# ARISE-Initiative/robosuite

Measured on AMD Instinct MI355X. Metric: env-steps/sec (whole node), Lift/Panda/OSC_POSE @4096 envs/GPU, higher is better.
Workload: dtype f32

## Files before the change

include/rsim.h:

```cpp
#ifndef RSIM_H
#define RSIM_H
#include <stddef.h>
#include <stdint.h>

#ifdef __cplusplus
extern "C" {
#endif

typedef struct rsim_model rsim_model;
typedef struct rsim_batch rsim_batch;

enum rsim_ctrl_type { RSIM_CTRL_OSC_POSE = 0, RSIM_CTRL_OSC_POSITION = 1, RSIM_CTRL_JOINT_POSITION = 2, RSIM_CTRL_JOINT_TORQUE = 3, RSIM_CTRL_JOINT_VELOCITY = 4 };
#define RSIM_JNT_MAX 16
typedef struct rsim_ctrl_desc {
  int32_t ndof;
  int32_t qpos_idx[RSIM_JNT_MAX];
  int32_t dof_idx[RSIM_JNT_MAX];
  int32_t act_idx[RSIM_JNT_MAX];
  int32_t eef_site;
  int32_t base_site;
  float kp[RSIM_JNT_MAX];
  float damping_ratio;
  float input_min[RSIM_JNT_MAX], input_max[RSIM_JNT_MAX], output_min[RSIM_JNT_MAX], output_max[RSIM_JNT_MAX];
  int32_t uncouple_pos_ori;
// ... 113 lines not shown
int rsim_sync(rsim_batch* b);
int rsim_observe(rsim_batch* b);

int rsim_set_episode(rsim_batch* b, int horizon);
int rsim_set_reset_bank(rsim_batch* b, int n_episodes, int n_patch, const int32_t* patch_idx, const float* bank);
int rsim_refill_reset_bank(rsim_batch* b, int n, const int32_t* env, const int32_t* episode, const float* rows);
int rsim_bank_poll_begin(rsim_batch* b);
int rsim_bank_poll(rsim_batch* b, int32_t* ep_index, int wait);
int rsim_refill_reset_bank_async(rsim_batch* b, int n, const int32_t* env, const int32_t* episode, const float* rows);
int rsim_bank_flush(rsim_batch* b);
int rsim_param_offset(const rsim_batch* b, const char* field, int elem);

int rsim_set_schedule(rsim_batch* b, int longest_first);
int rsim_set_applied_forces(rsim_batch* b, int enable);
int rsim_set_early_end(rsim_batch* b, int rules, int min_steps);
int rsim_end_episodes(rsim_batch* b, const uint8_t* mask_dev);
int rsim_set_stream_groups(rsim_batch* b, int groups);
void* rsim_group_stream(rsim_batch* b, int group);

int rsim_profile(rsim_batch* b, int enable, unsigned long long* out, int n_out);
int rsim_wavelog(rsim_batch* b, unsigned long long* out);
int rsim_profile_env(rsim_batch* b, int env);
int rsim_tier_snapshot(rsim_batch* b, int* host_tier);
const char* rsim_tuning_defaults(void);
int rsim_tier_stats(rsim_batch* b, unsigned long long* out2);
int rsim_pairlog(rsim_batch* b, unsigned long long* out);

int rsim_get_array(rsim_batch* b, int field, void* host_dst, size_t count);
int rsim_set_array(rsim_batch* b, int field, const void* host_src, size_t count);
void* rsim_device_ptr(rsim_batch* b, int field, size_t* count);
void* rsim_stream(rsim_batch* b);

int rsim_jac_site(rsim_batch* b, int env, int site, double* jacp, double* jacr);
int rsim_jac_body(rsim_batch* b, int env, int body, double* jacp, double* jacr);

int rsim_full_M(rsim_batch* b, int env, double* M);
typedef struct rsim_contact {
  double dist, pos[3], frame[9], friction[5], normal_force;
  int32_t geom1, geom2, dim, efc_address;
} rsim_contact;
int rsim_contacts(rsim_batch* b, int env, int max_out, rsim_contact* out);

int rsim_model_param_set(rsim_batch* b, const char* field, int env0, int nenv, const double* values, size_t count_per_env);

int rsim_model_param_get(rsim_batch* b, const char* field, int env0, int nenv, double* values, size_t count_per_env);

// ... 25 lines not shown
```

robosuite_amd/backend.py:

```python
from __future__ import annotations

import ctypes as C
import os

import numpy as np

from . import mjcf

_HERE = os.path.dirname(os.path.abspath(__file__))
LIB_PATH = os.environ.get("RSIM_LIB", os.path.join(_HERE, "librsim_hip.so"))
_LIB = None

FIELDS = ["qpos", "qvel", "qacc_warmstart", "ctrl", "time", "cstate", "xpos", "xquat", "qM", "qfrc_bias", "qfrc_passive", "qfrc_actuator",
          "qfrc_constraint", "qacc", "cdof", "rootcom", "contact", "efc_force", "ncon", "nefc", "niter", "obs", "reward", "success", "done", "ep_step",
          "ep_index", "diverged", "overflow", "bank_stale", "terminal_obs", "sensordata", "task_object", "cap_need", "qfrc_applied", "polish",
          "xfrc_applied"]
EXTRA_FIELDS = ["end_reason"]
FIELD_ID = {n: i for i, n in enumerate(FIELDS + EXTRA_FIELDS)}
END_REASONS = {"running": 0, "horizon": 1, "success": 2, "diverged": 3, "requested": 4}
INT_FIELDS = {"end_reason", "polish", "ncon", "nefc", "niter", "success", "done", "ep_step", "ep_index", "diverged", "overflow", "bank_stale", "task_object", "cap_need"}
CON_REC = 24
CSTATE = 32
OBS_MAX = 128
OBS_KINDS = {"qpos": 0, "cos": 1, "sin": 2, "qvel": 3, "qacc": 4, "site_pos": 5, "body_quat": 6, "site_quat": 7, "body_pos": 8, "body_minus_site": 9, "body_minus_body": 10,
# ... 195 lines not shown
        L.rsim_get_array.argtypes = [vp, C.c_int, vp, C.c_size_t]
        L.rsim_set_array.argtypes = [vp, C.c_int, vp, C.c_size_t]
        L.rsim_device_ptr.restype = vp
        L.rsim_device_ptr.argtypes = [vp, C.c_int, C.POINTER(C.c_size_t)]
        L.rsim_stream.restype = vp
        L.rsim_stream.argtypes = [vp]
        L.rsim_jac_site.argtypes = [vp, C.c_int, C.c_int, vp, vp]
        L.rsim_jac_body.argtypes = [vp, C.c_int, C.c_int, vp, vp]
        L.rsim_model_param_set.argtypes = [vp, C.c_char_p, C.c_int, C.c_int, vp, C.c_size_t]
        L.rsim_model_param_get.argtypes = [vp, C.c_char_p, C.c_int, C.c_int, vp, C.c_size_t]
        L.rsim_profile.argtypes = [vp, C.c_int, vp, C.c_int]
        L.rsim_wavelog.argtypes = [vp, vp]
        L.rsim_pairlog.argtypes = [vp, vp]
        L.rsim_set_schedule.argtypes = [vp, C.c_int]
        L.rsim_set_applied_forces.argtypes = [vp, C.c_int]
        L.rsim_set_stream_groups.argtypes = [vp, C.c_int]
        if hasattr(L, "rsim_set_early_end"):
            L.rsim_set_early_end.argtypes = [vp, C.c_int, C.c_int]
            L.rsim_end_episodes.argtypes = [vp, vp]
        L.rsim_group_stream.restype = vp; L.rsim_group_stream.argtypes = [vp, C.c_int]
        L.rsim_profile_env.argtypes = [vp, C.c_int]
        L.rsim_tier_snapshot.argtypes = [vp, vp]
        L.rsim_tier_stats.argtypes = [vp, vp]
        L.rsim_tuning_defaults.restype = C.c_char_p
        L.rsim_name2id.argtypes = [vp, C.c_char_p, C.c_char_p]
        L.rsim_id2name.argtypes = [vp, C.c_char_p, C.c_int]; L.rsim_id2name.restype = C.c_char_p
        L.rsim_full_M.argtypes = [vp, C.c_int, vp]
        L.rsim_contacts.argtypes = [vp, C.c_int, C.c_int, vp]
        L.rsim_comm_unique_id.argtypes = [vp, C.c_size_t]
        L.rsim_comm_create.argtypes = [vp, C.c_size_t, C.c_int, C.c_int, C.c_int, C.POINTER(vp)]
        L.rsim_allreduce_stats.argtypes = [vp, vp, C.c_int, C.c_int]
        L.rsim_comm_free.argtypes = [vp]; L.rsim_comm_free.restype = None
        _LIB = L
    return _LIB


def _chk(rc):
    if rc != 0:
        raise RsimError(lib().rsim_last_error().decode())


def tuning_sha16() -> str:
    import hashlib
    return hashlib.sha256(lib().rsim_tuning_defaults()).hexdigest()[:16]


# ... 296 lines not shown
                self._held.popleft()

    def _step_streams(self):
        import torch

        key = getattr(self, "_ngroups", 1)
        if getattr(self, "_ext_key", None) != key:
            ptrs = [self.group_stream(g) for g in range(key)] if key > 1 else [self.stream()]
            self._ext, self._ext_key = [torch.cuda.ExternalStream(p, device=f"cuda:{self.device}") for p in ptrs], key
        return self._ext

    PROFILE_SLOTS = ("load", "kin", "com", "crb", "broad", "narrow", "makec", "vel", "ctrl", "act", "solve", "euler", "store",
                     "n_sub", "n_cand", "n_con", "n_efc", "n_newton", "n_ls", "boxbox", "mpr", "plane", "n_boxbox", "n_mpr", "n_support",
                     "x0", "x1", "x2", "x3", "x4", "x5", "x6", "x7", "x8", "x9")

    def profile_env(self, env=-1):
        _chk(self._L.rsim_profile_env(self.ptr, int(env)))

    def tier_snapshot(self):
        out = np.zeros(self.B, dtype=np.int32)
        _chk(self._L.rsim_tier_snapshot(self.ptr, out.ctypes.data))
        return out

    def tier_stats(self):
        out = np.zeros(2, dtype=np.uint64)
        _chk(self._L.rsim_tier_stats(self.ptr, out.ctypes.data))
        return int(out[0]), int(out[1])

    def wavelog(self):
        out = np.zeros((self.B, 8), dtype=np.uint64)
        _chk(self._L.rsim_wavelog(self.ptr, out.ctypes.data))
        return out

    def set_applied_forces(self, enable=True):
        _chk(self._L.rsim_set_applied_forces(self.ptr, int(bool(enable))))

    def set_early_end(self, success=False, diverged=False, min_steps=1):
        _chk(self._L.rsim_set_early_end(self.ptr, (1 if success else 0) | (2 if diverged else 0), int(min_steps)))

    def end_episodes(self, mask):
        import torch

        if not isinstance(mask, torch.Tensor) or not mask.is_cuda or tuple(mask.shape) != (self.B,):
            raise RsimError(f"end_episodes: mask must be a CUDA tensor of shape ({self.B},)")
        m8 = (mask != 0).to(torch.uint8).contiguous()
        ev = torch.cuda.Event()
# ... 79 lines not shown
```

robosuite_amd/csrc/rsim_api.cpp:

```cpp
#include <hip/hip_runtime.h>
#include <dlfcn.h>
#include <rccl/rccl.h>
#include <math.h>
#include <stdarg.h>
#include <stdio.h>
#include <stdlib.h>
#include <string.h>

#include <algorithm>
#include <map>
#include <string>
#include <vector>

#include "../../include/rsim.h"
#include "rsim_internal.h"

#define RSIM_NCFG 5
#define RSIM_MAX_GROUPS 32
extern "C" int rsim_launch_step_cfg0(const DModel* m, const DBatch* b, const float* actions, int n_sub, int flags, hipStream_t stream);
extern "C" int rsim_launch_ctrl_reset_cfg0(const DModel* m, const DBatch* b, const unsigned char* mask, hipStream_t stream);
extern "C" int rsim_limits_cfg0(int* lim);
extern "C" int rsim_launch_step_cfg1(const DModel* m, const DBatch* b, const float* actions, int n_sub, int flags, hipStream_t stream);
extern "C" int rsim_launch_ctrl_reset_cfg1(const DModel* m, const DBatch* b, const unsigned char* mask, hipStream_t stream);
extern "C" int rsim_limits_cfg1(int* lim);
// ... 111 lines not shown
  int* d_patch;
  float* d_ft_base;
  float* d_ft;
  float* d_ft0;
  float* d_mesh;
  unsigned char* d_mask;
  DModel dm;
  DBatch db;
  void* fptr[RSIM_FIELD_COUNT];
  size_t fcount[RSIM_FIELD_COUNT];
  int fis_int[RSIM_FIELD_COUNT];
  int lim[10];
  int cfg;
  int cs;
  int* d_order;
  unsigned* d_cost;
  void* d_cm;
  size_t cm_bytes;
  int cm_dirty;
  DCtrl cm_ctrl;
  int tier;
  int lim_w[10];
  int* d_tier[2];
  int tier_flip;
  int share_cm;
  void* d_cm_w;
  size_t cm_bytes_w;
  int* d_wlist[2];
  int* d_wcount;
  hipStream_t wstream;
  hipEvent_t wfork, wjoin;
  int have_cost;
  int* d_order2[2];
  unsigned* d_cost2[2];
  long nstep;
  int schedule;
  int applied;
  int early_rules, early_min_steps;
  int* d_end_reason;
  int* d_seen_diverged;
  int* d_end_sel;
  int ended_outside;
  int groups, ngroups, forked;
  hipStream_t gstream[RSIM_MAX_GROUPS];
  hipEvent_t gev[RSIM_MAX_GROUPS], mev;
  hipStream_t bstream;
// ... 638 lines not shown
  dm.newton_polish_tol = getenv("RSIM_POLISH_TOL") ? (float)atof(getenv("RSIM_POLISH_TOL")) : 1.0f;
  dm.newton_polish_gate = getenv("RSIM_POLISH_GATE") ? (float)atof(getenv("RSIM_POLISH_GATE")) : 0.0f;
  dm.newton_exact = getenv("RSIM_NEWTON_EXACT") ? atoi(getenv("RSIM_NEWTON_EXACT")) : 1;
  dm.newton_ng = getenv("RSIM_NEWTON_NG") ? (float)atof(getenv("RSIM_NEWTON_NG")) : RSIM_NEWTON_NG;
  if (m->multijoint) { int r = fail("rsim_batch_create: bodies with more than one joint are not supported by the fused kernel"); delete b; return r; }
  if (m->D("jnt_stiffness")) for (int j = 0; j < m->njnt; j++) if (m->D("jnt_stiffness")[j] != 0.0) {
    int r = fail("rsim_batch_create: joint %d has a spring (stiffness %g): passive joint springs are not implemented in the fused kernel (tendon springs are)", j, m->D("jnt_stiffness")[j]);
    delete b; return r;
  }

  if (m->maxcondim > 4) { int r = fail("rsim_batch_create: condim %d contacts are not supported by the compiled kernel configuration (max 4)", m->maxcondim); delete b; return r; }
  for (int j = 0; j < m->njnt; j++) if (m->I("jnt_type")[j] == 1) { int r = fail("rsim_batch_create: ball joints are not supported by the fused kernel"); delete b; return r; }
  if (dalloc(&b->d_lt, m->lanetab.size())) return 1;
  HIPCHK(hipMemcpy(b->d_lt, m->lanetab.data(), m->lanetab.size() * sizeof(int), hipMemcpyHostToDevice));
  dm.lt = b->d_lt; dm.kin_rounds = m->kin_rounds; dm.ndynroot = m->ndynroot; dm.maxcondim = m->maxcondim;
  for (int r = 0; r < RSIM_MAXDYNROOT; r++) dm.dynroot[r] = r < m->ndynroot ? m->dynroot[r] : 0;
  dm.ft0 = b->d_ft0; dm.fenv = 0;
  dm.it = b->d_it; dm.ft = b->d_ft; dm.mesh_vert = b->d_mesh; dm.fstride = b->per_env ? (int)fs : 0;
  memcpy(dm.io, m->io, sizeof(dm.io));
  memcpy(dm.fo, m->fo, sizeof(dm.fo));
  dm.ctrl = m->ctrl;
  b->cs = m->ctrl.enabled ? m->ctrl.cs_size : RSIM_CS_SIZE;
  dm.ctrl.cs_size = b->cs;
  b->tier = TIER_NONE;
  if (b->cs <= RSIM_CS_LDS && !getenv("RSIM_NO_TIERS") && b->cfg <= 3) {
    int lw[10];
    if (b->cfg <= 2) k_limits_w[b->cfg](lw);
    else k_limits[5](lw);
    if (config_holds(m, lw)) { b->tier = b->cfg <= 2 ? TIER_FUSED : TIER_LIST; memcpy(b->lim_w, lw, sizeof(lw)); }
  }
  {
    auto jg_need = [](const int* lim) -> size_t {
      if (!(lim[9] & 4)) return 0;
      return (size_t)lim[6] * (size_t)(lim[2] + 1) + ((lim[9] & 8) ? (size_t)lim[2] * (size_t)(lim[2] + 1) : 0) + ((lim[9] & 16) ? (size_t)lim[5] * 22 : 0);
    };
    size_t jgf = jg_need(b->lim);
    if (b->tier != TIER_NONE) jgf = std::max(jgf, jg_need(b->lim_w));
    b->db.jg_stride = (long long)jgf;
    if (jgf && dalloc(&b->db.jg, (size_t)B * jgf)) return 1;
  }
  b->d_tier[0] = b->d_tier[1] = nullptr; b->tier_flip = 0;
  b->share_cm = 0; b->d_cm_w = nullptr; b->cm_bytes_w = 0; b->d_wlist[0] = b->d_wlist[1] = nullptr; b->d_wcount = nullptr; b->wstream = nullptr; b->wfork = b->wjoin = nullptr;
  if (b->tier != TIER_NONE) {
    for (int k = 0; k < 2; k++) if (dalloc(&b->d_tier[k], (size_t)B)) return 1;
    if (dalloc(&b->db.tstat, (size_t)2)) return 1;
  }
// ... 269 lines not shown
  int e = rsim_launch_step_list_cfg5(&b->dm, &dw, actions, n_sub, flags, grid, stream);
  if (e) return fail("wide-tier kernel launch failed: %s", hipGetErrorString((hipError_t)e));
  return 0;
}

static int launch(rsim_batch* b, const float* actions, int n_sub, int flags) {
  const int WCN = 2 + 2 * RSIM_MAX_GROUPS;
  HIPCHK(hipSetDevice(b->device));
  if (sync_controller(b)) return 1;
  if (b->applied) flags |= RF_APPLIED;
  const bool tiered = b->tier != TIER_NONE && (flags & RF_EPISODE) && (flags & RF_CTRL) && !(flags & RF_DEBUG);
  b->db.tier_cur = tiered ? b->d_tier[b->tier_flip] : nullptr; b->db.tier_next = tiered ? b->d_tier[b->tier_flip ^ 1] : nullptr;
  const bool no_advance = b->cfg == 0 || b->cfg == 1;
  b->db.tier_up_con = getenv("RSIM_TIER_UP_CON") ? atoi(getenv("RSIM_TIER_UP_CON")) : (no_advance ? 0 : 2);
  b->db.tier_up_efc = getenv("RSIM_TIER_UP_EFC") ? atoi(getenv("RSIM_TIER_UP_EFC")) : (no_advance ? 0 : 6);
  b->db.tier_pass = tiered ? 0 : -1; b->db.wlist = nullptr; b->db.wcount = nullptr; b->db.wlist2 = nullptr; b->db.wcount2 = nullptr;
  const bool fused = tiered && b->tier == TIER_FUSED, listed = tiered && b->tier == TIER_LIST;
  if (fused) {
    b->db.tier_con = b->lim[5]; b->db.tier_efc = b->lim[6];
    if (const char* e = getenv("RSIM_FORCE_HANDOVER")) b->db.tier_pass = 100 + atoi(e);
  }
  const bool grouped = (flags & RF_EPISODE) && (flags & RF_CTRL) && b->ngroups > 1;
  const bool early = (flags & RF_EPISODE) && b->early_rules && b->db.bank;
  if (!grouped || b->cm_dirty || memcmp(&b->cm_ctrl, &b->dm.ctrl, sizeof(DCtrl))) { if (join_groups(b)) return 1; }
  if (ensure_constants(b)) return 1;
  if ((flags & RF_OBS) && !b->dm.task.enabled) return fail("the task (observation / reward epilogue) was configured after the batch was created");
  if ((flags & RF_CTRL) && !b->dm.ctrl.enabled) return fail("no controller configured (rsim_model_set_controller)");
  b->db.order = nullptr; b->db.cost = nullptr;
  if (grouped) {
    if (fork_groups(b)) return 1;
    const bool sched = b->schedule && b->d_order;
    for (int g = 0; g < b->ngroups; g++) {
      const int e0 = (int)((long long)b->B * g / b->ngroups), e1 = (int)((long long)b->B * (g + 1) / b->ngroups);
      DBatch db = b->db;
      db.env0 = e0; db.nenv = e1 - e0;
      if (sched) {
        if (b->have_cost) {
          int eo = rsim_launch_order(b->d_cost + e0, b->d_order + e0, e1 - e0, b->gstream[g]);
          if (eo) return fail("dispatch-order kernel launch failed: %s", hipGetErrorString((hipError_t)eo));
          db.order = b->d_order + e0;
        }
        db.cost = b->d_cost;
      }
      if (listed) {
        int* cnt = b->d_wcount + b->tier_flip * WCN + 2 + 2 * g;
        int el = rsim_launch_tier_list(b->db.tier_cur, b->d_wlist[0] + e0, cnt, b->d_wcount + (b->tier_flip ^ 1) * WCN + 2 + 2 * g, e0, e1 - e0, b->gstream[g]);
        if (el) return fail("tier-list kernel launch failed: %s", hipGetErrorString((hipError_t)el));
        db.wlist2 = b->d_wlist[1] + e0; db.wcount2 = cnt + 1;
      }
      int e = k_step_launch[b->cfg](&b->dm, &db, actions, n_sub, flags, b->gstream[g]);
      if (e) return fail("kernel launch failed: %s", hipGetErrorString((hipError_t)e));
      if (listed) {
        int* cnt = b->d_wcount + b->tier_flip * WCN + 2 + 2 * g;
        if (wide_pass(b, actions, n_sub, flags, 1, b->d_wlist[0] + e0, cnt, b->gstream[g])) return 1;
        if (wide_pass(b, actions, n_sub, flags, 2, b->d_wlist[1] + e0, cnt + 1, b->gstream[g])) return 1;
      }
      if (early && end_episodes_launch(b, e0, e1 - e0, nullptr, 0, (flags & (RF_APPLIED | RF_DEBUG)) ? 1 : 0, b->gstream[g])) return 1;
      if (b->db.bank && (b->db.horizon > 0 || early)) {
        db.order = nullptr; db.cost = nullptr;
        if (b->db.bank_P > 0 && b->db.cm_stride) {
          e = k_prepare_launch[b->cfg](&b->dm, &db, e1 - e0, 1, b->gstream[g]);
          if (e) return fail("constant-block kernel launch failed: %s", hipGetErrorString((hipError_t)e));
        }
        if (b->dm.task.enabled) {
          db.tier_cur = nullptr; db.tier_next = nullptr; db.tier_pass = -1; db.wlist = nullptr; db.wcount = nullptr; db.wlist2 = nullptr; db.wcount2 = nullptr;
          e = k_reset_obs_launch[b->cfg](&b->dm, &db, b->gstream[g]);
          if (e) return fail("reset-observation kernel launch failed: %s", hipGetErrorString((hipError_t)e));
        }
      }
    }
    if (sched) b->have_cost = 1;
    if (tiered) b->tier_flip ^= 1;
    b->gen++;
    b->derived_stale = 1;
    return 0;
  }
  const bool sched1 = (flags & RF_EPISODE) && (flags & RF_CTRL) && b->schedule && b->d_order;
  const int cur = (int)(b->nstep & 1), prev = cur ^ 1;
  const bool traced = sched1_trace(flags);
  if (traced) tr_mark(b, 0);
  if (sched1) {
// ... 9 lines not shown
    int* cnt = b->d_wcount + b->tier_flip * WCN;
    HIPCHK(hipEventRecord(b->wfork, b->stream));
    HIPCHK(hipStreamWaitEvent(b->wstream, b->wfork, 0));
    int el = rsim_launch_tier_list(b->db.tier_cur, b->d_wlist[0], cnt, b->d_wcount + (b->tier_flip ^ 1) * WCN, 0, b->B, b->wstream);
    if (el) return fail("tier-list kernel launch failed: %s", hipGetErrorString((hipError_t)el));
    if (wide_pass(b, actions, n_sub, flags, 1, b->d_wlist[0], cnt, b->wstream)) return 1;
    HIPCHK(hipEventRecord(b->wjoin, b->wstream));
    b->db.wlist2 = b->d_wlist[1]; b->db.wcount2 = cnt + 1;
  }
  if (traced) tr_mark(b, 2);
  int e = k_step_launch[b->cfg](&b->dm, &b->db, actions, n_sub, flags, b->stream);
  if (e) return fail("kernel launch failed: %s", hipGetErrorString((hipError_t)e));
  if (traced) tr_mark(b, 3);
  if (listed) {
    HIPCHK(hipStreamWaitEvent(b->stream, b->wjoin, 0));
    if (traced) tr_mark(b, 4);
    if (wide_pass(b, actions, n_sub, flags, 2, b->d_wlist[1], b->d_wcount + b->tier_flip * WCN + 1, b->stream)) return 1;
  } else if (traced) tr_mark(b, 4);
  if (tiered) b->tier_flip ^= 1;
  if (traced) tr_mark(b, 5);
  if (sched1) b->nstep++;
  if (early && end_episodes_launch(b, 0, b->B, nullptr, 0, (flags & (RF_APPLIED | RF_DEBUG)) ? 1 : 0, b->stream)) return 1;
  if ((flags & RF_EPISODE) && b->db.bank && (b->db.horizon > 0 || early)) {
    if (b->db.bank_P > 0 && b->db.cm_stride) {
      e = k_prepare_launch[b->cfg](&b->dm, &b->db, b->B, 1, b->stream);
      if (e) return fail("constant-block kernel launch failed: %s", hipGetErrorString((hipError_t)e));
    }
    if (traced) tr_mark(b, 6);
    if (b->dm.task.enabled) {
      DBatch db2 = b->db;
      db2.order = nullptr; db2.cost = nullptr;
      db2.tier_cur = nullptr; db2.tier_next = nullptr; db2.tier_pass = -1; db2.wlist = nullptr; db2.wcount = nullptr; db2.wlist2 = nullptr; db2.wcount2 = nullptr;
      e = k_reset_obs_launch[b->cfg](&b->dm, &db2, b->stream);
      if (e) return fail("reset-observation kernel launch failed: %s", hipGetErrorString((hipError_t)e));
    }
    if (traced) tr_mark(b, 7);
  }
  b->gen++;
  b->derived_stale = (flags & RF_DEBUG) ? 0 : 1;
  return 0;
}
static bool derived_field(int f) { return (f >= RSIM_XPOS && f <= RSIM_NITER) || f == RSIM_SENSORDATA; }
extern "C" int rsim_forward(rsim_batch* b);
static int refresh_forward(rsim_batch* b) {
  DBatch keep = b->db;
  b->db.overflow = nullptr; b->db.cap_need = nullptr; b->db.mprc = nullptr; b->db.bpl = nullptr;
  const int r = launch(b, nullptr, 1, RF_POSVEL | RF_ACTSOLVE | RF_DEBUG | RF_NOSTORE);
  b->db.overflow = keep.overflow; b->db.cap_need = keep.cap_need; b->db.mprc = keep.mprc; b->db.bpl = keep.bpl;
  return r;
}
static int refresh_derived(rsim_batch* b, int field) { return (derived_field(field) && b->derived_stale) ? refresh_forward(b) : 0; }
extern "C" int rsim_forward(rsim_batch* b) { return launch(b, nullptr, 1, RF_POSVEL | RF_ACTSOLVE | RF_DEBUG); }
// ... 300 lines not shown
  static const char* const envs[] = {"RSIM_NEWTON_NS", "RSIM_NEWTON_NA", "RSIM_NEWTON_LS", "RSIM_NEWTON_NG", "RSIM_NEWTON_WIDE", "RSIM_NEWTON_EXACT", "RSIM_NEWTON_REFINE",
                                     "RSIM_POLISH_TOL", "RSIM_POLISH_GATE", "RSIM_BP_REACH", "RSIM_NEAR_THRESH", "RSIM_NEAR_GAIN", "RSIM_MPR_CONE", "RSIM_NO_MPR_WARMSTART", "RSIM_NO_MPR_PORTAL_WARMSTART",
                                     "RSIM_TIER_UP_CON", "RSIM_TIER_UP_EFC", "RSIM_NO_TIERS", "RSIM_NO_SHARE_CM", "RSIM_EULER_FULL", "RSIM_FORCE_HANDOVER"};
  for (const char* e : envs) if (const char* v = getenv(e)) { s += ";env:"; s += e; s += "="; s += v; }
  return s.c_str();
}
extern "C" int rsim_tier_stats(rsim_batch* b, unsigned long long* out2) {
  if (!out2) return fail("rsim_tier_stats: null destination");
  out2[0] = out2[1] = 0;
  if (b->tier == TIER_NONE) return 0;
  HIPCHK(hipSetDevice(b->device));
  if (join_groups(b)) return 1;
  HIPCHK(hipStreamSynchronize(b->stream));
  HIPCHK(hipMemcpy(out2, b->db.tstat, 2 * sizeof(unsigned long long), hipMemcpyDeviceToHost));
  return 0;
}
extern "C" int rsim_tier_snapshot(rsim_batch* b, int* host_tier) {
  if (!host_tier) return fail("rsim_tier_snapshot: null destination");
  HIPCHK(hipSetDevice(b->device));
  if (b->tier == TIER_NONE) { memset(host_tier, 0, (size_t)b->B * sizeof(int)); return 0; }
  if (join_groups(b)) return 1;
  HIPCHK(hipStreamSynchronize(b->stream));
  HIPCHK(hipMemcpy(host_tier, b->d_tier[b->tier_flip], (size_t)b->B * sizeof(int), hipMemcpyDeviceToHost));
  return 0;
}

extern "C" int rsim_wavelog(rsim_batch* b, unsigned long long* out) { if (join_groups(b)) return 1;
  if (!b->db.prof) return fail("rsim_wavelog: profiling is not enabled");
  HIPCHK(hipSetDevice(b->device));
  HIPCHK(hipStreamSynchronize(b->stream));
  HIPCHK(hipMemcpy(out, b->db.prof + RP_COUNT, 8 * (size_t)b->B * sizeof(unsigned long long), hipMemcpyDeviceToHost));
  return 0;
}

extern "C" void* rsim_device_ptr(rsim_batch* b, int field, size_t* count) {
  if (field < 0 || field >= RSIM_FIELD_COUNT) { fail("bad field id %d", field); return nullptr; }
  if (count) *count = b->fcount[field];
  if (refresh_derived(b, field)) return nullptr;
  return b->fptr[field];
}
extern "C" int rsim_get_array(rsim_batch* b, int field, void* dst, size_t count) { if (join_groups(b)) return 1;
  if (field < 0 || field >= RSIM_FIELD_COUNT) return fail("bad field id %d", field);
  if (count > b->fcount[field]) return fail("rsim_get_array: count %zu > field size %zu", count, b->fcount[field]);
  if (refresh_derived(b, field)) return 1;
  HIPCHK(hipSetDevice(b->device));
  HIPCHK(hipStreamSynchronize(b->stream));
// ... 272 lines not shown
```

robosuite_amd/csrc/rsim_internal.h:

```cpp
#pragma once
#include <stdint.h>

enum {
  IO_body_parentid, IO_body_rootid, IO_body_jntadr, IO_body_jntnum, IO_body_dofadr, IO_body_dofnum, IO_body_depth,
  IO_body_mocap, IO_body_moving, IO_body_ancmask , IO_body_dofmask , IO_body_isroot,
  IO_jnt_type, IO_jnt_qposadr, IO_jnt_dofadr, IO_jnt_bodyid, IO_jnt_limited,
  IO_dof_bodyid, IO_dof_jntid, IO_dof_ancmask , IO_dof_cvelmask , IO_dof_zerodot,
  IO_cg_geomid, IO_cg_type, IO_cg_bodyid, IO_cg_condim, IO_cg_priority, IO_cg_meshadr, IO_cg_meshnum,
  IO_pair_g1, IO_pair_g2,
  IO_site_bodyid,
  IO_act_trnid, IO_act_biastype, IO_act_ctrllimited, IO_act_forcelimited,
  IO_tendon_adr, IO_tendon_num, IO_tendon_limited, IO_wrap_dof, IO_wrap_qadr, IO_eq_tendon,
  IO_sensor_type , IO_sensor_site, IO_sensor_adr ,
  IO_COUNT
};
enum {
  FO_body_pos, FO_body_quat, FO_body_ipos, FO_body_iquat, FO_body_mass, FO_body_inertia, FO_body_invweight0, FO_body_subtreemass,
  FO_jnt_pos, FO_jnt_axis, FO_jnt_range, FO_jnt_margin, FO_jnt_solref, FO_jnt_solimp, FO_qpos0,
  FO_dof_armature, FO_dof_damping, FO_dof_frictionloss, FO_dof_solref, FO_dof_solimp, FO_dof_invweight0,
  FO_cg_size, FO_cg_pos, FO_cg_quat, FO_cg_friction, FO_cg_solref, FO_cg_solimp, FO_cg_solmix, FO_cg_margin, FO_cg_gap,
  FO_cg_rbound, FO_cg_rcenter, FO_cg_aabb ,
  FO_cg_capsule ,
  FO_site_pos, FO_site_quat,
  FO_act_gear, FO_act_gainprm, FO_act_biasprm, FO_act_ctrlrange, FO_act_forcerange,
// ... 191 lines not shown
#define RSIM_NEWTON_NA 1e-5f
#define RSIM_NEWTON_NG 0.f
#endif

enum { RP_LOAD, RP_KIN, RP_COM, RP_CRB, RP_BROAD, RP_NARROW, RP_MAKEC, RP_VEL, RP_CTRL, RP_ACT, RP_SOLVE, RP_EULER, RP_STORE,
       RP_N_SUB, RP_N_CAND, RP_N_CON, RP_N_EFC, RP_N_NEWTON, RP_N_LS, RP_BOXBOX, RP_MPR, RP_PLANE, RP_N_BOXBOX, RP_N_MPR, RP_N_SUPPORT,
       RP_X0, RP_X1, RP_X2, RP_X3, RP_X4, RP_X5, RP_X6, RP_X7, RP_X8, RP_X9,  RP_COUNT };

struct DDr { float density, viscosity, pos, quat, inertia, mass, friction, solref, solimp, frictionloss, damping, armature;
             unsigned long long body_mask, geom_mask, joint_mask; };

enum {
  RF_POSVEL = 1,
  RF_CTRL = 2,
  RF_SETGOAL = 4,
  RF_ACTSOLVE = 8,
  RF_INTEGRATE = 16,
  RF_DEBUG = 32,
  RF_OBS = 64,
  RF_EPISODE = 128,
  RF_RESET_ONLY = 256,
  RF_NOSTORE = 512,
  RF_APPLIED = 1024,
};
```

robosuite_amd/csrc/rsim_step.hip:

```cpp
#include <hip/hip_runtime.h>
#include <stdint.h>
#include <type_traits>

#include "../../include/rsim.h"
#include "rsim_internal.h"

#ifndef RSIM_CFG
#define RSIM_CFG 0
#endif
#if RSIM_CFG == 0
#define RSIM_DIMS 32, 16, 16, 24, 16, 16, 64, 192
#define RSIM_SYM(x) x##_cfg0
#define RSIM_DIMS_W 32, 16, 16, 24, 16, 32, 128, 192
#elif RSIM_CFG == 1
#define RSIM_DIMS 32, 16, 32, 24, 16, 32, 64, 192
#define RSIM_SYM(x) x##_cfg1
#define RSIM_DIMS_W 32, 16, 32, 24, 16, 32, 128, 192
#elif RSIM_CFG == 2
#define RSIM_DIMS 64, 16, 16, 32, 32, 32, 64, 320
#define RSIM_SYM(x) x##_cfg2
#define RSIM_DIMS_W 64, 16, 16, 32, 32, 32, 128, 320
#elif RSIM_CFG == 3
#define RSIM_DIMS 64, 32, 48, 64, 32, 32, 128, 640
#define RSIM_SYM(x) x##_cfg3
// ... 3874 lines not shown
      }
      if (lane == 0 && t.task == 1) {
        const V3 cube = ld3(sm.xpos + 3 * t.object_body), grip = ld3(sm.spos + 3 * t.grip_site);
        const bool succ = cube.z > t.table_height + t.lift_margin;
        float r = 0.f;
        if (succ) r = 2.25f;
        else if (t.reward_shaping) { r = 1.f - tanhf(10.f * norm(cube - grip)); if (grasp) r += 0.25f; }
        if (reward) { *reward = r * t.reward_scale / 2.25f; *success = succ ? 1 : 0; }
      }
    }
  }

  __device__ __forceinline__ void fwd_constraint() {
    if (sm.nefc == 0) {
      if (lane < m.nv) { sm.qacc[lane] = sm.qacc_smooth[lane]; sm.qfrc_constraint[lane] = 0.f; }
      if (lane == 0) sm.niter = 0;
      SYNC();
      return;
    }
    solve_newton();
  }
};

struct Handover { int sub0; float time; bool fresh_ctrl, handed; int ndiverged, need_con, need_efc; float cstate; unsigned t_launch; };

template <int NB, int NJ, int NV, int NG, int NS, int NCON, int NEFC, int NPAIR, bool DBG, int FUSED = 0>
__device__ __forceinline__ bool step_body(const DModel& m, const DBatch& b, const float* __restrict__ actions, int n_sub, int flags, int slot, Handover* ho = nullptr) {
  typedef Smem<NB, NJ, NV, NG, NS, NCON, NEFC, NPAIR> SM;
  const int lane = threadIdx.x;
  const int tpass = (!DBG && b.tier_cur) ? (FUSED == 2 ? 2 : FUSED == 1 ? 0 : b.tier_pass) : -1;
  const bool resume = FUSED == 2 && ho->sub0 > 0;
  if ((tpass <= 0 || FUSED) && slot >= (b.nenv ? b.nenv : b.B)) return false;
  const int env = uni((tpass > 0 && !FUSED) ? b.wlist[slot] : (b.order ? b.order[slot] : slot) + b.env0);
  if ((flags & RF_RESET_ONLY) && !b.needs_reset[env]) return false;
  if (!FUSED && tpass == 0 && b.tier_cur[env] != 0) return false;
  const unsigned t_launch = resume ? ho->t_launch : (b.cost ? (unsigned)uni((int)(clock64() >> 6)) : 0u);
  const float* fp = m.ft + (size_t)env * m.fstride;
  Sim<SM> sim(m, fp, lane, b.prof, b.cm, b.cm_stride ? (const char*)b.cm_env + (size_t)env * b.cm_stride : (const char*)b.cm);
  sim.pf.acc = b.prof_env == -1 || b.prof_env == env;
  if (b.prof) sim.pf.pairs = b.prof + RP_COUNT + 8 * (size_t)b.B;
  sim.pf.start();
  if (b.prof && lane == 0 && !resume) {
    unsigned long long* wl = b.prof + RP_COUNT + 8 * (size_t)env;
    wl[0] = (unsigned)__builtin_amdgcn_s_getreg((31 << 11) | 4);
    wl[1] = (unsigned)__builtin_amdgcn_s_getreg((31 << 11) | 20);
    wl[2] = wall_clock64();
  }
  if (!resume) {
    for (int i = lane; i < m.nq; i += 64) sm.qpos[i] = b.qpos[(size_t)env * m.nq + i];
    for (int i = lane; i < m.nv; i += 64) { sm.qvel[i] = b.qvel[(size_t)env * m.nv + i]; sm.qacc_ws[i] = b.qacc_ws[(size_t)env * m.nv + i]; }
    if (lane >= m.nv && lane < NV) { sm.qvel[lane] = 0.f; sm.qacc_ws[lane] = 0.f; sm.qacc[lane] = 0.f; }
    for (int i = lane; i < m.nu; i += 64) sm.ctrl[i] = b.ctrl[(size_t)env * m.nu + i];
  }
  const int cs = m.ctrl.cs_size, csl = cs < RSIM_CS_LDS ? cs : RSIM_CS_LDS;
  sim.cst = (gwf)(b.cstate + (size_t)env * cs);
  if (b.bpl) sim.bpl = (int __attribute__((address_space(1)))*)(b.bpl + (size_t)env * 320);
  if (b.mprc) { sim.mprc = (gwf)(b.mprc + (size_t)env * Sim<SM>::MPRC * m.npair); sim.mpr_portal = b.mprc_portal != 0; }
  if constexpr (Sim<SM>::JG) sim.Jg = (gwf)(b.jg + (size_t)env * b.jg_stride);
  if constexpr (Sim<SM>::MG) sim.Mg = sim.Jg + SM::NEFC_ * SM::JS_;
// ... 131 lines not shown
    const bool done = b.horizon > 0 && st >= b.horizon;
    if (done && b.bank) {
      const int ep = b.ep_index[env] + 1, slot = ep % b.bank_E;
      const float* src = b.bank + ((size_t)env * b.bank_E + slot) * (m.nq + b.bank_P);
      if (lane == 0 && b.bank_tag && b.bank_tag[(size_t)env * b.bank_E + slot] != ep) b.bank_stale[env] += 1;
      if (b.term_obs && m.task.enabled) for (int i = lane; i < m.task.nobs; i += 64) b.term_obs[(size_t)env * m.task.nobs + i] = b.obs[(size_t)env * m.task.nobs + i];
      SYNC();
      for (int i = lane; i < m.nq; i += 64) sm.qpos[i] = src[i];
      if (lane < NV) { sm.qvel[lane] = 0.f; sm.qacc_ws[lane] = 0.f; sm.ctrl[lane] = 0.f; }
      for (int p2 = lane; p2 < b.bank_P; p2 += 64) {
        const int pi = b.patch_idx[p2];
        if (pi < 0) { b.task_object[env] = (int)src[m.nq + p2]; continue; }
        b.ft_rw[(size_t)env * m.fstride + pi] = src[m.nq + p2];
        if (b.ft_base) b.ft_base[(size_t)env * m.fstride + pi] = src[m.nq + p2];
      }
      time = 0.f;
      st = 0;
      if (sim.mprc) for (int p2 = lane; p2 < m.npair; p2 += 64) sim.mprc[Sim<SM>::MPRC * p2 + 3] = 0.f;
      if (DBG || (flags & RF_APPLIED)) {
        for (int i = lane; i < m.nv; i += 64) b.qfrc_applied[(size_t)env * m.nv + i] = 0.f;
        for (int i = lane; i < m.nbody * 6; i += 64) b.xfrc_applied[(size_t)env * m.nbody * 6 + i] = 0.f;
      }
      if (lane == 0) { b.ep_index[env] = ep; b.needs_reset[env] = 1; }
      SYNC();
    }
    if (lane == 0) { b.done[env] = done ? 1 : 0; b.ep_step[env] = st; }
  }
  if (!DBG || !(flags & RF_NOSTORE)) {
    for (int i = lane; i < m.nq; i += 64) b.qpos[(size_t)env * m.nq + i] = sm.qpos[i];
    for (int i = lane; i < m.nv; i += 64) { b.qvel[(size_t)env * m.nv + i] = sm.qvel[i]; b.qacc_ws[(size_t)env * m.nv + i] = sm.qacc_ws[i]; }
    for (int i = lane; i < m.nu; i += 64) b.ctrl[(size_t)env * m.nu + i] = sm.ctrl[i];
    if (lane < csl) sim.cst[lane] = sm.cstate[lane];
    if (lane == 0) b.time[env] = time;
  }
  if (b.overflow && lane == 0 && sim.ovf) b.overflow[env] += sim.ovf;
  if (b.cap_need && lane == 0) { int* cn = b.cap_need + 2 * (size_t)env; if (sim.need_con > cn[0]) cn[0] = sim.need_con; if (sim.need_efc > cn[1]) cn[1] = sim.need_efc; }
  if (b.cost && lane == 0) {
    unsigned cst = (unsigned)(clock64() >> 6) - t_launch;
    if (sim.near_sep < m.near_thresh) cst += (unsigned)((float)cst * m.near_gain);
    b.cost[env] = cst;
  }
  if (b.prof && lane == 0) {
    unsigned long long* wl = b.prof + RP_COUNT + 8 * (size_t)env;
    wl[3] = wall_clock64(); wl[4] = sim.pf.c_mpr; wl[5] = sim.pf.c_support; wl[6] = sim.pf.c_newton; wl[7] = sim.pf.c_cand;
  }
  if constexpr (DBG) if (flags & RF_DEBUG) {
    const int nb = m.nbody, nv = m.nv;
    for (int i = lane; i < nb * 3; i += 64) { b.xpos[(size_t)env * nb * 3 + i] = sm.xpos[i]; b.rootcom[(size_t)env * nb * 3 + i] = sm.rootcom[3 * sim.cm->broot[i / 3] + i % 3]; }
    for (int i = lane; i < nb * 4; i += 64) b.xquat[(size_t)env * nb * 4 + i] = sm.xquat[i];
    for (int e = lane; e < nv * nv; e += 64) { int i = e / nv, j = e - i * nv; b.qM[(size_t)env * nv * nv + e] = sim.Mrd(i * SM::NVP + j); }
    for (int e = lane; e < nv * 6; e += 64) b.cdof[(size_t)env * nv * 6 + e] = sm.cdof[(e / 6) * 9 + e % 6];
    for (int i = lane; i < nv; i += 64) {
      size_t o = (size_t)env * nv + i;
      b.qfrc_bias[o] = sm.qfrc_bias[i]; b.qfrc_passive[o] = sm.qfrc_passive[i];
      if (flags & RF_ACTSOLVE) { b.qfrc_actuator[o] = sm.qfrc_actuator[i]; b.qfrc_constraint[o] = sm.qfrc_constraint[i]; b.qacc[o] = sm.qacc[i]; }
    }
    int ncon = sm.ncon;
    sim.csync();
    for (int c = lane; c < ncon; c += 64) {
      float* r = b.contact + ((size_t)env * NCON + c) * RSIM_CON_REC;
// ... 8 lines not shown
      for (int i = lane; i < sm.nefc; i += 64) b.efc_force[(size_t)env * NEFC + i] = sm.e_force[i];
    if (lane == 0) { b.ncon[env] = ncon; b.nefc[env] = sm.nefc; b.niter[env] = sm.niter; if (b.polish) b.polish[env] = sm.polish; }
  }
  return false;
}

#ifdef RSIM_WAVES_PER_EU
#define RSIM_KSTEP_ATTR __attribute__((amdgpu_waves_per_eu(RSIM_WAVES_PER_EU, RSIM_WAVES_PER_EU)))
#else
#define RSIM_KSTEP_ATTR
#endif
template <int NB, int NJ, int NV, int NG, int NS, int NCON, int NEFC, int NPAIR>
__global__ RSIM_KSTEP_ATTR __launch_bounds__(64, RSIM_MINWAVES) void k_step(DModel m, DBatch b, const float* __restrict__ actions, int n_sub, int flags) {
#ifdef RSIM_DIMS_W
  typedef const char __attribute__((address_space(4)))* ka_t;
  ka_t ka = (ka_t)__builtin_amdgcn_kernarg_segment_ptr();
  constexpr size_t b_off = (sizeof(DModel) + alignof(DBatch) - 1) & ~(alignof(DBatch) - 1);
  const DModel& mk = *(const DModel*)(const DModel __attribute__((address_space(4)))*)ka;
  const DBatch& bk = *(const DBatch*)(const DBatch __attribute__((address_space(4)))*)(ka + b_off);
#define m mk
#define b bk
  const int slot = (int)blockIdx.x;
  Handover ho;
  ho.sub0 = 0; ho.time = 0.f; ho.fresh_ctrl = false; ho.handed = false; ho.ndiverged = 0; ho.need_con = 0; ho.need_efc = 0; ho.cstate = 0.f; ho.t_launch = 0u;
  bool wide = false;
  if (b.tier_cur) {
    if (slot >= (b.nenv ? b.nenv : b.B)) return;
    wide = b.tier_cur[uni((b.order ? b.order[slot] : slot) + b.env0)] != 0;
  }
  if (!wide) {
    const int over = uni(step_body<NB, NJ, NV, NG, NS, NCON, NEFC, NPAIR, false, 1>(m, b, actions, n_sub, flags, slot, &ho) ? 1 : 0);
    if (!over) return;
    ho.sub0 = uni(ho.sub0); ho.time = __builtin_bit_cast(float, uni(__builtin_bit_cast(int, ho.time))); ho.fresh_ctrl = uni(ho.fresh_ctrl ? 1 : 0) != 0; ho.handed = true;
    ho.ndiverged = uni(ho.ndiverged); ho.need_con = uni(ho.need_con); ho.need_efc = uni(ho.need_efc); ho.t_launch = (unsigned)uni((int)ho.t_launch);
  }
  step_body<RSIM_DIMS_W, false, 2>(m, b, actions, n_sub, flags, slot, &ho);
#undef m
#undef b
#else
  step_body<NB, NJ, NV, NG, NS, NCON, NEFC, NPAIR, false>(m, b, actions, n_sub, flags, (int)blockIdx.x);
#endif
}
template <int NB, int NJ, int NV, int NG, int NS, int NCON, int NEFC, int NPAIR>
__global__ __launch_bounds__(64, 1) void k_step_list(DModel m, DBatch b, const float* __restrict__ actions, int n_sub, int flags) {
  const int n = *b.wcount;
  for (int i = blockIdx.x; i < n; i += gridDim.x) {
    step_body<NB, NJ, NV, NG, NS, NCON, NEFC, NPAIR, false>(m, b, actions, n_sub, flags, i);
    __syncthreads();
  }
}
template <int NB, int NJ, int NV, int NG, int NS, int NCON, int NEFC, int NPAIR>
__global__ __launch_bounds__(64, 1) void k_step_dbg(DModel m, DBatch b, const float* __restrict__ actions, int n_sub, int flags) {
  step_body<NB, NJ, NV, NG, NS, NCON, NEFC, NPAIR, true>(m, b, actions, n_sub, flags, (int)blockIdx.x);
}
template <int NB, int NJ, int NV, int NG, int NS, int NCON, int NEFC, int NPAIR>
__global__ __launch_bounds__(64, 1) void k_reset_obs(DModel m, DBatch b) {
  step_body<NB, NJ, NV, NG, NS, NCON, NEFC, NPAIR, false>(m, b, nullptr, 1, RF_POSVEL | RF_ACTSOLVE | RF_OBS | RF_RESET_ONLY, (int)blockIdx.x);
}

// ... 203 lines not shown
```

Before: 1.289 million.

## Run episode reset and re-observation inside the fused step kernel

When an environment's episode restarts during the fused step, the kernel now loops back in the same workgroup. It rebuilds per-env constant blocks and re-runs a reset-only forward/observe pass, instead of the host launching separate prepare and reset kernels over the whole batch. This removes extra full-batch kernel launches and the passes that scan all environments only to act on the few being reset. It adds fences and scalar cache invalidation inside the kernel, plus extra code that may raise register pressure. An env var can restore the separate pass, and a debug API exposes the restart flags.

```diff
diff --git a/include/rsim.h b/include/rsim.h
--- a/include/rsim.h
+++ b/include/rsim.h
@@ -159,6 +159,7 @@
 int rsim_wavelog(rsim_batch* b, unsigned long long* out);
 int rsim_profile_env(rsim_batch* b, int env);
 int rsim_tier_snapshot(rsim_batch* b, int* host_tier);
+int rsim_restart_flags(rsim_batch* b, int* host_flags);
 const char* rsim_tuning_defaults(void);
 int rsim_tier_stats(rsim_batch* b, unsigned long long* out2);
 int rsim_pairlog(rsim_batch* b, unsigned long long* out);
diff --git a/robosuite_amd/backend.py b/robosuite_amd/backend.py
--- a/robosuite_amd/backend.py
+++ b/robosuite_amd/backend.py
@@ -241,6 +241,8 @@
         L.rsim_profile_env.argtypes = [vp, C.c_int]
         L.rsim_tier_snapshot.argtypes = [vp, vp]
         L.rsim_tier_stats.argtypes = [vp, vp]
+        if hasattr(L, "rsim_restart_flags"):
+            L.rsim_restart_flags.argtypes = [vp, vp]
         L.rsim_tuning_defaults.restype = C.c_char_p
         L.rsim_name2id.argtypes = [vp, C.c_char_p, C.c_char_p]
         L.rsim_id2name.argtypes = [vp, C.c_char_p, C.c_int]; L.rsim_id2name.restype = C.c_char_p
@@ -583,6 +585,11 @@
         _chk(self._L.rsim_tier_snapshot(self.ptr, out.ctypes.data))
         return out
 
+    def restart_flags(self):
+        out = np.zeros(self.B, dtype=np.int32)
+        _chk(self._L.rsim_restart_flags(self.ptr, out.ctypes.data))
+        return out
+
     def tier_stats(self):
         out = np.zeros(2, dtype=np.uint64)
         _chk(self._L.rsim_tier_stats(self.ptr, out.ctypes.data))
diff --git a/robosuite_amd/csrc/rsim_api.cpp b/robosuite_amd/csrc/rsim_api.cpp
--- a/robosuite_amd/csrc/rsim_api.cpp
+++ b/robosuite_amd/csrc/rsim_api.cpp
@@ -157,6 +157,7 @@
   int tier;
   int lim_w[10];
   int* d_tier[2];
+  int separate_reset;
   int tier_flip;
   int share_cm;
   void* d_cm_w;
@@ -841,6 +842,7 @@
   dm.ctrl = m->ctrl;
   b->cs = m->ctrl.enabled ? m->ctrl.cs_size : RSIM_CS_SIZE;
   dm.ctrl.cs_size = b->cs;
+  { const char* e = getenv("RSIM_SEPARATE_RESET_PASS"); b->separate_reset = (e && atoi(e) != 0) ? 1 : 0; }
   b->tier = TIER_NONE;
   if (b->cs <= RSIM_CS_LDS && !getenv("RSIM_NO_TIERS") && b->cfg <= 3) {
     int lw[10];
@@ -1156,6 +1158,8 @@
   }
   const bool grouped = (flags & RF_EPISODE) && (flags & RF_CTRL) && b->ngroups > 1;
   const bool early = (flags & RF_EPISODE) && b->early_rules && b->db.bank;
+  const bool inkernel = (b->lim[9] & 32) && !b->separate_reset && !early && (flags & RF_EPISODE) && (flags & RF_CTRL) && !(flags & RF_DEBUG);
+  if (inkernel) flags |= RF_RESET_INKERNEL;
   if (!grouped || b->cm_dirty || memcmp(&b->cm_ctrl, &b->dm.ctrl, sizeof(DCtrl))) { if (join_groups(b)) return 1; }
   if (ensure_constants(b)) return 1;
   if ((flags & RF_OBS) && !b->dm.task.enabled) return fail("the task (observation / reward epilogue) was configured after the batch was created");
@@ -1190,7 +1194,7 @@
         if (wide_pass(b, actions, n_sub, flags, 2, b->d_wlist[1] + e0, cnt + 1, b->gstream[g])) return 1;
       }
       if (early && end_episodes_launch(b, e0, e1 - e0, nullptr, 0, (flags & (RF_APPLIED | RF_DEBUG)) ? 1 : 0, b->gstream[g])) return 1;
-      if (b->db.bank && (b->db.horizon > 0 || early)) {
+      if (!inkernel && b->db.bank && (b->db.horizon > 0 || early)) {
         db.order = nullptr; db.cost = nullptr;
         if (b->db.bank_P > 0 && b->db.cm_stride) {
           e = k_prepare_launch[b->cfg](&b->dm, &db, e1 - e0, 1, b->gstream[g]);
@@ -1246,12 +1250,12 @@
   if (sched1) b->nstep++;
   if (early && end_episodes_launch(b, 0, b->B, nullptr, 0, (flags & (RF_APPLIED | RF_DEBUG)) ? 1 : 0, b->stream)) return 1;
   if ((flags & RF_EPISODE) && b->db.bank && (b->db.horizon > 0 || early)) {
-    if (b->db.bank_P > 0 && b->db.cm_stride) {
+    if (!inkernel && b->db.bank_P > 0 && b->db.cm_stride) {
       e = k_prepare_launch[b->cfg](&b->dm, &b->db, b->B, 1, b->stream);
       if (e) return fail("constant-block kernel launch failed: %s", hipGetErrorString((hipError_t)e));
     }
     if (traced) tr_mark(b, 6);
-    if (b->dm.task.enabled) {
+    if (!inkernel && b->dm.task.enabled) {
       DBatch db2 = b->db;
       db2.order = nullptr; db2.cost = nullptr;
       db2.tier_cur = nullptr; db2.tier_next = nullptr; db2.tier_pass = -1; db2.wlist = nullptr; db2.wcount = nullptr; db2.wlist2 = nullptr; db2.wcount2 = nullptr;
@@ -1598,6 +1602,14 @@
   if (join_groups(b)) return 1;
   HIPCHK(hipStreamSynchronize(b->stream));
   HIPCHK(hipMemcpy(host_tier, b->d_tier[b->tier_flip], (size_t)b->B * sizeof(int), hipMemcpyDeviceToHost));
+  return 0;
+}
+extern "C" int rsim_restart_flags(rsim_batch* b, int* host_flags) {
+  if (!host_flags) return fail("rsim_restart_flags: null destination");
+  HIPCHK(hipSetDevice(b->device));
+  if (join_groups(b)) return 1;
+  HIPCHK(hipStreamSynchronize(b->stream));
+  HIPCHK(hipMemcpy(host_flags, b->db.needs_reset, (size_t)b->B * sizeof(int), hipMemcpyDeviceToHost));
   return 0;
 }
 
diff --git a/robosuite_amd/csrc/rsim_internal.h b/robosuite_amd/csrc/rsim_internal.h
--- a/robosuite_amd/csrc/rsim_internal.h
+++ b/robosuite_amd/csrc/rsim_internal.h
@@ -237,4 +237,5 @@
   RF_RESET_ONLY = 256,
   RF_NOSTORE = 512,
   RF_APPLIED = 1024,
-};
+  RF_RESET_INKERNEL = 2048,
+};
diff --git a/robosuite_amd/csrc/rsim_step.hip b/robosuite_amd/csrc/rsim_step.hip
--- a/robosuite_amd/csrc/rsim_step.hip
+++ b/robosuite_amd/csrc/rsim_step.hip
@@ -3920,19 +3920,21 @@
   }
 };
 
-struct Handover { int sub0; float time; bool fresh_ctrl, handed; int ndiverged, need_con, need_efc; float cstate; unsigned t_launch; };
+struct Handover { int sub0; float time; bool fresh_ctrl, handed; int ndiverged, need_con, need_efc; float cstate; unsigned t_launch;
+                  bool restarted; };
 
 template <int NB, int NJ, int NV, int NG, int NS, int NCON, int NEFC, int NPAIR, bool DBG, int FUSED = 0>
 __device__ __forceinline__ bool step_body(const DModel& m, const DBatch& b, const float* __restrict__ actions, int n_sub, int flags, int slot, Handover* ho = nullptr) {
   typedef Smem<NB, NJ, NV, NG, NS, NCON, NEFC, NPAIR> SM;
-  const int lane = threadIdx.x;
-  const int tpass = (!DBG && b.tier_cur) ? (FUSED == 2 ? 2 : FUSED == 1 ? 0 : b.tier_pass) : -1;
+  const int lane = FUSED ? opaque_lane((int)threadIdx.x) : (int)threadIdx.x;
+  const bool reentry = FUSED == 1 && (flags & RF_RESET_ONLY);
+  const int tpass = (!DBG && b.tier_cur && !reentry) ? (FUSED == 2 ? 2 : FUSED == 1 ? 0 : b.tier_pass) : -1;
   const bool resume = FUSED == 2 && ho->sub0 > 0;
   if ((tpass <= 0 || FUSED) && slot >= (b.nenv ? b.nenv : b.B)) return false;
   const int env = uni((tpass > 0 && !FUSED) ? b.wlist[slot] : (b.order ? b.order[slot] : slot) + b.env0);
-  if ((flags & RF_RESET_ONLY) && !b.needs_reset[env]) return false;
+  if (!reentry && (flags & RF_RESET_ONLY) && !b.needs_reset[env]) return false;
   if (!FUSED && tpass == 0 && b.tier_cur[env] != 0) return false;
-  const unsigned t_launch = resume ? ho->t_launch : (b.cost ? (unsigned)uni((int)(clock64() >> 6)) : 0u);
+  const unsigned t_launch = resume ? ho->t_launch : ((b.cost && !reentry) ? (unsigned)uni((int)(clock64() >> 6)) : 0u);
   const float* fp = m.ft + (size_t)env * m.fstride;
   Sim<SM> sim(m, fp, lane, b.prof, b.cm, b.cm_stride ? (const char*)b.cm_env + (size_t)env * b.cm_stride : (const char*)b.cm);
   sim.pf.acc = b.prof_env == -1 || b.prof_env == env;
@@ -4110,6 +4112,7 @@
         for (int i = lane; i < m.nbody * 6; i += 64) b.xfrc_applied[(size_t)env * m.nbody * 6 + i] = 0.f;
       }
       if (lane == 0) { b.ep_index[env] = ep; b.needs_reset[env] = 1; }
+      if constexpr (FUSED != 0) ho->restarted = true;
       SYNC();
     }
     if (lane == 0) { b.done[env] = done ? 1 : 0; b.ep_step[env] = st; }
@@ -4123,7 +4126,7 @@
   }
   if (b.overflow && lane == 0 && sim.ovf) b.overflow[env] += sim.ovf;
   if (b.cap_need && lane == 0) { int* cn = b.cap_need + 2 * (size_t)env; if (sim.need_con > cn[0]) cn[0] = sim.need_con; if (sim.need_efc > cn[1]) cn[1] = sim.need_efc; }
-  if (b.cost && lane == 0) {
+  if (b.cost && !reentry && lane == 0) {
     unsigned cst = (unsigned)(clock64() >> 6) - t_launch;
     if (sim.near_sep < m.near_thresh) cst += (unsigned)((float)cst * m.near_gain);
     b.cost[env] = cst;
@@ -4178,19 +4181,38 @@
 #define b bk
   const int slot = (int)blockIdx.x;
   Handover ho;
-  ho.sub0 = 0; ho.time = 0.f; ho.fresh_ctrl = false; ho.handed = false; ho.ndiverged = 0; ho.need_con = 0; ho.need_efc = 0; ho.cstate = 0.f; ho.t_launch = 0u;
+  ho.sub0 = 0; ho.time = 0.f; ho.fresh_ctrl = false; ho.handed = false; ho.ndiverged = 0; ho.need_con = 0; ho.need_efc = 0; ho.cstate = 0.f; ho.t_launch = 0u; ho.restarted = false;
   bool wide = false;
   if (b.tier_cur) {
     if (slot >= (b.nenv ? b.nenv : b.B)) return;
     wide = b.tier_cur[uni((b.order ? b.order[slot] : slot) + b.env0)] != 0;
   }
-  if (!wide) {
-    const int over = uni(step_body<NB, NJ, NV, NG, NS, NCON, NEFC, NPAIR, false, 1>(m, b, actions, n_sub, flags, slot, &ho) ? 1 : 0);
-    if (!over) return;
-    ho.sub0 = uni(ho.sub0); ho.time = __builtin_bit_cast(float, uni(__builtin_bit_cast(int, ho.time))); ho.fresh_ctrl = uni(ho.fresh_ctrl ? 1 : 0) != 0; ho.handed = true;
-    ho.ndiverged = uni(ho.ndiverged); ho.need_con = uni(ho.need_con); ho.need_efc = uni(ho.need_efc); ho.t_launch = (unsigned)uni((int)ho.t_launch);
-  }
-  step_body<RSIM_DIMS_W, false, 2>(m, b, actions, n_sub, flags, slot, &ho);
+  const float* act = actions;
+  int nsub = n_sub, fl = flags;
+  for (;;) {
+    bool over = wide;
+    if (!wide) {
+      over = uni(step_body<NB, NJ, NV, NG, NS, NCON, NEFC, NPAIR, false, 1>(m, b, act, nsub, fl, slot, &ho) ? 1 : 0) != 0;
+      if (over) {
+        ho.sub0 = uni(ho.sub0); ho.time = __builtin_bit_cast(float, uni(__builtin_bit_cast(int, ho.time))); ho.fresh_ctrl = uni(ho.fresh_ctrl ? 1 : 0) != 0; ho.handed = true;
+        ho.ndiverged = uni(ho.ndiverged); ho.need_con = uni(ho.need_con); ho.need_efc = uni(ho.need_efc); ho.t_launch = (unsigned)uni((int)ho.t_launch);
+      }
+    }
+    if (over) step_body<RSIM_DIMS_W, false, 2>(m, b, act, nsub, fl, slot, &ho);
+    if (!(fl & RF_RESET_INKERNEL) || !uni(ho.restarted ? 1 : 0)) return;
+    __builtin_amdgcn_fence(__ATOMIC_RELEASE, "agent"); __builtin_amdgcn_wave_barrier(); __builtin_amdgcn_fence(__ATOMIC_ACQUIRE, "agent");
+    __builtin_amdgcn_s_dcache_inv();
+    if (b.cm_stride != 0 && b.bank_P > 0) {
+      const int env = uni((b.order ? b.order[slot] : slot) + b.env0);
+      char* const cmb = (char*)b.cm_env + (size_t)env * b.cm_stride;
+      Sim<Smem<NB, NJ, NV, NG, NS, NCON, NEFC, NPAIR>> ps(m, m.ft + (size_t)env * m.fstride, opaque_lane((int)threadIdx.x), nullptr, cmb, cmb);
+      ps.prepare_constants((cmw_t)cmb);
+      __builtin_amdgcn_fence(__ATOMIC_RELEASE, "agent"); __builtin_amdgcn_wave_barrier(); __builtin_amdgcn_fence(__ATOMIC_ACQUIRE, "agent");
+      __builtin_amdgcn_s_dcache_inv();
+    }
+    if (!m.task.enabled) return;
+    act = nullptr; nsub = 1; fl = RF_POSVEL | RF_ACTSOLVE | RF_OBS | RF_RESET_ONLY; wide = false;
+  }
 #undef m
 #undef b
 #else
```

Result: faster. 1.318 million (median of 6 runs) (+2.3%).
